# wgurecky/CORRLA_RS

Measured on AMD Instinct MI355X. Metric: RSVD GFLOP/s on 16k x 16k f32 rank-128, higher is better.
Workload: dtype f32

## Files before the change

### corrla_rs_amd/csrc/hip_backend.hpp

```cpp
#pragma once
#include <hip/hip_runtime.h>
#include <rccl/rccl.h>

#include <cmath>
#include <cstdio>
#include <cstdlib>
#include <cstring>
#include <limits>
#include <random>
#include <string>
#include <type_traits>
#include <vector>

#include "core_svd_plan.hpp"
#include "driver.hpp"
#include "hip_kernels.hpp"
#include "tsqr_kernels.hpp"
#include "jacobi_mc_kernels.hpp"
#include "ata_kernels.hpp"
#include "tall_kernels.hpp"
#include "mixed_kernels.hpp"
#include "grad_kernels.hpp"
#include "knn2_kernels.hpp"
#include "grad_wide_kernels.hpp"
#include "spmm_kernels.hpp"

namespace corrla {

#define CORRLA_HIP(call)                                                                                       \
  do {                                                                                                         \
    hipError_t e_ = (call);                                                                                    \
    if (e_ != hipSuccess)                                                                                      \
      throw Error(ST_EHIP, std::string(#call) + " failed: " + hipGetErrorString(e_) + " (" __FILE__ ":" +       \
                               std::to_string(__LINE__) + ")");                                                \
  } while (0)
#define CORRLA_NCCL(call)                                                                                      \
  do {                                                                                                         \
    ncclResult_t r_ = (call);                                                                                  \
    if (r_ != ncclSuccess) throw Error(ST_ECOMM, std::string(#call) + " failed: " + ncclGetErrorString(r_));   \
  } while (0)

inline int env_int(const char* name, int dflt) {
  const char* v = std::getenv(name);
  return v && *v ? std::atoi(v) : dflt;
}

template <class T>
struct NcclType;
template <>
struct NcclType<float> {
  static constexpr ncclDataType_t v = ncclFloat;
};
template <>
struct NcclType<double> {
  static constexpr ncclDataType_t v = ncclDouble;
};

class HipDev {
 public:
  int device = 0;
  int num_cus = 256;
  hipStream_t stream = nullptr;
  ncclComm_t comm = nullptr;
  int comm_rank = 0, comm_size = 1;
  int n_collectives = 0;
  double collective_bytes = 0;

  explicit HipDev(int dev_ordinal) : device(dev_ordinal) {
    int count = 0;
    if (hipGetDeviceCount(&count) != hipSuccess || count <= 0)
      throw Error(ST_ENODEV, "no HIP device visible (libcorrla_rsvd has no CPU fallback)");
    if (dev_ordinal < 0 || dev_ordinal >= count) throw Error(ST_EINVAL, "device ordinal out of range");
    CORRLA_HIP(hipSetDevice(device));
    hipDeviceProp_t prop;
    CORRLA_HIP(hipGetDeviceProperties(&prop, device));
    if (std::strncmp(prop.gcnArchName, "gfx950", 6) != 0)
      throw Error(ST_ENODEV, std::string("device is ") + prop.gcnArchName + ", this library is built for gfx950 only");
    num_cus = prop.multiProcessorCount;
    CORRLA_HIP(hipStreamCreateWithFlags(&stream, hipStreamNonBlocking));
    CORRLA_HIP(hipMalloc(&zero_page_, 256));
    CORRLA_HIP(hipHostMalloc(&pinned_, kPinnedBytes, hipHostMallocDefault));
    for (auto& e : events_) CORRLA_HIP(hipEventCreate(&e));
    CORRLA_HIP(hipMemsetAsync(zero_page_, 0, 256, stream));
    set_lds_limits();
    {
      std::random_device rd;
      entropy_ = ((uint64_t)rd() << 32) ^ (uint64_t)rd();
    }
    no_device_chol_ = env_int("CORRLA_HOST_CHOL", 0) != 0;
    jmc_min_l_ = env_int("CORRLA_JMC_MIN_L", 96);
    jmc_max_b_ = std::min(32, std::max(2, env_int("CORRLA_JMC_MAX_B", 24)));
    robust_passes_ = std::max(2, env_int("CORRLA_ROBUST_PASSES", 2));
    robust_qr_ = env_int("CORRLA_DEVICE_ROBUST_QR", 1) != 0;
    gemm_debug_flags_ = env_int("CORRLA_GEMM_DEBUG", 0);
    gemm_knobs_.split_nn = env_int("CORRLA_SPLIT_NN", 0);
    gemm_knobs_.split_tn = env_int("CORRLA_SPLIT_TN", 0);
    gemm_knobs_.mw = env_int("CORRLA_MW", 0);
    gemm_knobs_.xcd_remap = env_int("CORRLA_GEMM_XCD", 1);
    gemm_knobs_.tall_min_rows = env_int("CORRLA_TALL_MIN_ROWS", 65536);
    gemm_knobs_.persist_max_tiles = env_int("CORRLA_GEMM_PERSIST_TILES", 16);
    gemm_knobs_.f64_waves = env_int("CORRLA_F64_WAVES", 8);
    if (const char* e = std::getenv("CORRLA_MIXED_MIN_WORK")) gemm_knobs_.mixed_min_work = std::atof(e);
    gemm_knobs_.even_blocks = env_int("CORRLA_EVEN_BLOCKS", 0) != 0;
    gemm_knobs_.no_gram_alias = env_int("CORRLA_NO_GRAM_ALIAS", 0) != 0;
    gemm_knobs_.no_rotate = env_int("CORRLA_GEMM_NO_ROTATE", 0) != 0;
    gemm_knobs_.mixed_split = env_int("CORRLA_MIXED_SPLIT", 0);
  }
  ~HipDev() {
    (void)hipSetDevice(device);
    if (stream) (void)hipStreamSynchronize(stream);
    if (comm) (void)ncclCommDestroy(comm);
    for (auto& c : chunks_) (void)hipFree(c.p);
    for (auto& c : zchunks_) (void)hipFree(c.p);
    if (zero_page_) (void)hipFree(zero_page_);
    if (pinned_) (void)hipHostFree(pinned_);
    for (auto& e : events_)
      if (e) (void)hipEventDestroy(e);
    for (auto& e : ev_pool_) (void)hipEventDestroy(e);
    if (stream) (void)hipStreamDestroy(stream);
  }
  HipDev(const HipDev&) = delete;
  HipDev& operator=(const HipDev&) = delete;

  int nranks() const { return comm_size; }

  uint64_t fresh_seed(bool rank_invariant) {
    uint64_t z = (rank_invariant ? 0x5eedull : entropy_) + 0x9e3779b97f4a7c15ull * (uint64_t)(++(rank_invariant ? calls_sharded_ : calls_));
    z = (z ^ (z >> 30)) * 0xbf58476d1ce4e5b9ull;
    z = (z ^ (z >> 27)) * 0x94d049bb133111ebull;
    z ^= z >> 31;
    return z ? z : 0x5eedull;
  }

  void comm_init(const void* id128, int rank, int nranks_) {
    CORRLA_HIP(hipSetDevice(device));
    ncclUniqueId id;
    static_assert(sizeof(ncclUniqueId) <= CORRLA_UNIQUE_ID_BYTES, "unique id size");
    std::memcpy(&id, id128, sizeof(id));
    if (comm) {
      (void)ncclCommDestroy(comm);
      comm = nullptr;
    }
    CORRLA_NCCL(ncclCommInitRank(&comm, nranks_, id, rank));
    comm_rank = rank;
    comm_size = nranks_;
  }
  void comm_info(int* rank_out, int* nranks_out) {
    if (!comm) {
      *rank_out = 0;
      *nranks_out = 0;
      return;
    }
    CORRLA_NCCL(ncclCommUserRank(comm, rank_out));
    CORRLA_NCCL(ncclCommCount(comm, nranks_out));
  }

  void begin_call() {
    CORRLA_HIP(hipSetDevice(device));
    events_set_[0] = events_set_[1] = events_set_[2] = false;
    n_collectives = 0;
    collective_bytes = 0;
    marks_.clear();
    ev_used_ = 0;
    phase_mark(nullptr);
    for (auto& c : chunks_) c.used = 0;
    sp_scratch_ = nullptr;
    sp_scratch_bytes_ = 0;
    for (auto& c : zchunks_) {
      c.zeroed = std::min<size_t>(c.used, (size_t)256 << 20);
      c.used = 0;
      if (c.zeroed) CORRLA_HIP(hipMemsetAsync(c.p, 0, c.zeroed, stream));
    }
// ... 337 lines not shown
    sync();
    for (size_t i = 0; i < n; ++i) host[i] = (double)tmp[i];
  }
  template <class T>
  void upload_skinny(const double* host, int64_t rows, int64_t cols, int64_t ld_host, Skinny<T>& dst) {
    const size_t n = (size_t)dst.ld * dst.cols_alloc;
    std::vector<T> heap;
    T* tmp = (T*)pinned_;
    if (n * sizeof(T) > kPinnedBytes) {
      heap.resize(n);
      tmp = heap.data();
    }
    sync();
    std::memset(tmp, 0, n * sizeof(T));
    for (int64_t j = 0; j < cols; ++j)
      for (int64_t i = 0; i < rows; ++i) tmp[(size_t)j * dst.ld + i] = (T)host[(size_t)j * ld_host + i];
    CORRLA_HIP(hipMemcpyAsync(dst.p, tmp, n * sizeof(T), hipMemcpyHostToDevice, stream));
    if (!heap.empty()) sync();
  }
  template <class T>
  void upload_skinny_native(const T* host, int64_t ld_host, Skinny<T>& dst) {
    h2d_2d(dst.p, dst.ld, host, ld_host, dst.rows, dst.cols);
  }
  template <class T>
  void copy_in_skinny(const T* src_dev, int64_t ld_src, Skinny<T>& dst) {
    CORRLA_HIP(hipMemcpy2DAsync(dst.p, (size_t)dst.ld * sizeof(T), src_dev, (size_t)ld_src * sizeof(T),
                                (size_t)dst.rows * sizeof(T), (size_t)dst.cols, hipMemcpyDeviceToDevice, stream));
  }
  template <class T>
  void copy_skinny(const Skinny<T>& src, Skinny<T>& dst) {
    CORRLA_HIP(hipMemcpyAsync(dst.p, src.p, (size_t)src.ld * src.cols_alloc * sizeof(T), hipMemcpyDeviceToDevice, stream));
  }
  template <class T>
  void copy_cols(const Skinny<T>& src, Skinny<T>& dst, int64_t c0, int64_t n) {
    if (src.ld != dst.ld) throw Error(ST_EINVAL, "internal: copy_cols needs equal leading dimensions");
    if (n > 0)
      CORRLA_HIP(hipMemcpyAsync(dst.p + c0 * dst.ld, src.p, (size_t)n * src.ld * sizeof(T), hipMemcpyDeviceToDevice, stream));
  }
  template <class T>
  void sub_inplace(Skinny<T>& y, const Skinny<T>& p) {
    const int64_t n = y.ld * std::min(y.cols_alloc, p.cols_alloc);
    const int blocks = (int)std::min<int64_t>(4096, std::max<int64_t>(1, (n + 255) / 256));
    hipLaunchKernelGGL((k::sub_kernel<T>), dim3(blocks), dim3(256), 0, stream, y.p, (const T*)p.p, n);
    CORRLA_HIP(hipGetLastError());
  }
  template <class T>
  void zero_cols(Skinny<T>& s, int64_t c0, int64_t c1) {
    if (c1 > c0) memset_zero(s.p + c0 * s.ld, (size_t)(c1 - c0) * s.ld * sizeof(T));
  }
  template <class T>
  void store_values(const T* host_src, int64_t n, T* dst, bool dst_is_host) {
    if (dst_is_host) {
      std::memcpy(dst, host_src, sizeof(T) * n);
    } else {
      CORRLA_HIP(hipMemcpyAsync(dst, host_src, sizeof(T) * n, hipMemcpyHostToDevice, stream));
      sync();
    }
  }
  template <class T>
  void copy_values_out(const T* src_dev, int64_t n, T* dst, bool dst_is_host) {
    CORRLA_HIP(hipMemcpyAsync(dst, src_dev, sizeof(T) * n, dst_is_host ? hipMemcpyDeviceToHost : hipMemcpyDeviceToDevice,
                              stream));
    if (dst_is_host) sync();
  }
  template <class T>
  bool device_chol_fits(int64_t l) const {
    return l <= 4096 && k::chol_inv_fits((int)l, sizeof(T)) && !no_device_chol_;
  }
  template <class T>
  bool device_chol_blocked_fits(int64_t l) const {
    const int64_t n1 = round_up((l + 1) / 2, (int64_t)4);
    return l > 8 && l <= 4096 && k::chol_inv_fits((int)n1, sizeof(T)) && !no_device_chol_;
  }
  template <class T>
  void copy_block(const Skinny<T>& src, int64_t r0, int64_t c0, int64_t rows, int64_t cols, Skinny<T>& dst, int64_t dr0,
                  int64_t dc0) {
    if (rows <= 0 || cols <= 0) return;
    CORRLA_HIP(hipMemcpy2DAsync(dst.p + dc0 * dst.ld + dr0, (size_t)dst.ld * sizeof(T), src.p + c0 * src.ld + r0,
                                (size_t)src.ld * sizeof(T), (size_t)rows * sizeof(T), (size_t)cols, hipMemcpyDeviceToDevice,
                                stream));
  }
  template <class T>
  void chol_inv(const Skinny<T>& g, int64_t r, T piv_rel, Skinny<T>& m_out, void* st_dev, int slot) {
    hipLaunchKernelGGL((k::chol_inv_kernel<T>), dim3(1), dim3(k::chol_inv_threads((int)r)),
                       k::chol_inv_lds_bytes((int)r, sizeof(T)), stream, (const T*)g.p, g.ld, (int)r, piv_rel, m_out.p,
                       m_out.ld, (k::CholStatus*)st_dev + slot);
    CORRLA_HIP(hipGetLastError());
  }
  void set_run_if(const int* p) { run_if_ = p; }
  int robust_passes() const { return robust_passes_; }
  void set_robust_passes(int n) { robust_passes_ = n; }
  bool svd_more_sweeps() {
    if (jmc_extra_sweeps_ >= 24) return false;
    jmc_extra_sweeps_ += 8;
    jmc_sweeps_hint_ = 0;
    return true;
  }
  bool svd_force_v() {
    if (jmc_force_v_) return false;
    jmc_force_v_ = true;
    return true;
  }
  void svd_sweeps_used(int n) { jmc_sweeps_hint_ = std::max(jmc_sweeps_hint_ - 1, n); }
  int* alloc_flags(int n) { return (int*)alloc_zeroed(sizeof(int) * (size_t)std::max(n, 1)); }
  void* alloc_zeroed_bytes(size_t bytes) { return alloc_zeroed(bytes); }
  void read_bytes(const void* dev_p, size_t bytes, void* host) {
    CORRLA_HIP(hipMemcpyAsync(host, dev_p, bytes, hipMemcpyDeviceToHost, stream));
    sync();
  }
  template <class T>
  void poison_entry(Skinny<T>& s, int64_t i, int64_t j, int kind) {
    hipLaunchKernelGGL((k::poison_entry_kernel<T>), dim3(1), dim3(1), 0, stream, s.p + j * s.ld + i, kind);
    CORRLA_HIP(hipGetLastError());
  }
  struct ArenaMark {
    std::vector<size_t> used, zused;
  };
  ArenaMark arena_mark() const {
    ArenaMark mk;
    for (const auto& c : chunks_) mk.used.push_back(c.used);
    for (const auto& c : zchunks_) mk.zused.push_back(c.used);
    return mk;
  }
  void arena_rewind(const ArenaMark& mk) {
    sp_scratch_ = nullptr;
    sp_scratch_bytes_ = 0;
    for (size_t i = 0; i < chunks_.size(); ++i) chunks_[i].used = i < mk.used.size() ? mk.used[i] : 0;
    for (size_t i = 0; i < zchunks_.size(); ++i) {
      Chunk& c = zchunks_[i];
      const size_t keep = i < mk.zused.size() ? mk.zused[i] : 0;
      if (c.used > keep) CORRLA_HIP(hipMemsetAsync((char*)c.p + keep, 0, c.used - keep, stream));
      c.zeroed = std::max(c.zeroed, c.used);
      c.used = keep;
    }
  }
  int sharded_handshake(int local_status) {
    if (comm_size <= 1 && !(comm && env_int("CORRLA_FORCE_ALLREDUCE", 0))) return local_status;
    if (!comm) throw Error(ST_ECOMM, "communicator not initialised");
    double h[8] = {(double)local_status, (double)robust_passes_, (double)jmc_extra_sweeps_, (double)jmc_sweeps_hint_,
                   jmc_force_v_ ? 1.0 : 0.0, 0.0, 0.0, 0.0};
    double* d = (double*)alloc_bytes(sizeof(h));
    CORRLA_HIP(hipMemcpyAsync(d, h, sizeof(h), hipMemcpyHostToDevice, stream));
    CORRLA_NCCL(ncclAllReduce(d, d, 8, ncclDouble, ncclMax, comm, stream));
    ++n_collectives;
    collective_bytes += sizeof(h);
    CORRLA_HIP(hipMemcpyAsync(h, d, sizeof(h), hipMemcpyDeviceToHost, stream));
    sync();
    robust_passes_ = (int)h[1];
    jmc_extra_sweeps_ = (int)h[2];
    jmc_sweeps_hint_ = (int)h[3];
    jmc_force_v_ = h[4] != 0.0;
    return (int)h[0];
  }
  void read_flags(const int* dev_p, int n, int* host) {
    CORRLA_HIP(hipMemcpyAsync(host, dev_p, sizeof(int) * (size_t)n, hipMemcpyDeviceToHost, stream));
    sync();
  }
  template <class T>
  bool device_qr_robust_fits(int64_t l) const {
    return robust_qr_ && (device_chol_fits<T>(l) || device_chol_blocked_fits<T>(l));
  }
  bool qr_inplace_fits(int64_t l) const { return col_blocking(l).nblk == 1; }
  template <class T>
  void* alloc_inspect() { return alloc_zeroed(sizeof(k::GramInspect<T>)); }
  template <class T>
  const void* inspect_shift_ptr(const void* insp) const { return &((const k::GramInspect<T>*)insp)->shift; }
  template <class T>
  void gram_inspect(Skinny<T>& g, int64_t l, float shift_rel, int shift_mode, void* insp) {
    hipLaunchKernelGGL((k::gram_inspect_kernel<T>), dim3(1), dim3(1024), 0, stream, g.p, g.ld, (int)l, shift_rel, shift_mode,
                       (k::GramInspect<T>*)insp, run_if_);
    CORRLA_HIP(hipGetLastError());
  }
  template <class T>
  void combine_need(int* need, const void* insp, const int* na, const int* nb) {
    hipLaunchKernelGGL((k::combine_need_kernel<T>), dim3(1), dim3(1), 0, stream, need, (const k::GramInspect<T>*)insp, na, nb,
                       run_if_);
    CORRLA_HIP(hipGetLastError());
  }
  template <class T>
  void chol_inv_robust(const Skinny<T>& g, int64_t r, T piv_rel, float shift_rel, int shift_mode, float null_excess,
                       Skinny<T>& m_out, void* st_dev, int slot, int* need_next, int* null_mask,
                       const void* abs_shift = nullptr, float need_ratio = 0.f) {
    k::CholRobust rb{shift_rel, shift_mode, null_excess, need_next, null_mask, run_if_, need_ratio, abs_shift};
    hipLaunchKernelGGL((k::chol_inv_kernel<T>), dim3(1), dim3(k::chol_inv_threads((int)r)),
                       k::chol_inv_lds_bytes((int)r, sizeof(T)), stream, (const T*)g.p, g.ld, (int)r, piv_rel, m_out.p,
                       m_out.ld, (k::CholStatus*)st_dev + slot, rb);
    CORRLA_HIP(hipGetLastError());
  }
  template <class T>
  void apply_inplace(Skinny<T>& y, int64_t l, const Skinny<T>& m) {
    Skinny<T> out = y.view_cols(l);
    Skinny<T> mv = m.view_cols(l);
    mv.rows = l;
    launch_gemm<T>(true, as_rowmajor_transposed(y, l), mv, out, (const T*)nullptr);
  }
  template <class T>
  void refill_null(Skinny<T>& y, int64_t l, const int* null_mask, uint64_t seed) {
    const int bx = (int)std::min<int64_t>(64, (y.rows + 255) / 256);
    hipLaunchKernelGGL((k::refill_null_kernel<T>), dim3((unsigned)std::max(bx, 1), (unsigned)l), dim3(256), 0, stream, y.p, y.ld,
                       y.rows, (int)l, null_mask, seed, run_if_);
    CORRLA_HIP(hipGetLastError());
  }

  void read_chol_status(const void* st_dev, int n, int* fail, float* min_ratio, float* dev_i) {
    static_assert(sizeof(k::CholStatus) == 32, "driver.hpp assumes 32-byte status records");
    static_assert(k::kNeedNonFinite == kFlagNonFinite && k::kNeedNullCols == kFlagNullCols, "need_next bits: kernels vs driver");
    std::vector<k::CholStatus> h((size_t)std::max(n, 1));
    CORRLA_HIP(hipMemcpyAsync(h.data(), st_dev, sizeof(k::CholStatus) * n, hipMemcpyDeviceToHost, stream));
    sync();
    for (int i = 0; i < n; ++i) {
      fail[i] = h[i].fail;
      min_ratio[i] = h[i].min_ratio;
      dev_i[i] = h[i].dev_i;
      if (env_int("CORRLA_DEBUG", 0) >= 2)
        std::fprintf(stderr, "[corrla] chol_inv[%d]: fail %d min_ratio %.3g dev_i %.3g clk %lld wall %lld (%.0f MHz)\n", i,
                     h[i].fail, h[i].min_ratio, h[i].dev_i, h[i].clk, h[i].wall,
                     h[i].wall > 0 ? 100.0 * (double)h[i].clk / (double)h[i].wall : 0.0);
    }
  }

  template <class T>
  void inv_sqrt_series(Skinny<T>& g, int64_t r, Skinny<T>& m_out) {
    Skinny<T> e2 = alloc_skinny<T>(r, r), e3 = alloc_skinny<T>(r, r);
    if (e2.ld != g.ld || m_out.ld != g.ld) throw Error(ST_EINVAL, "internal: series operands must share a leading dimension");
    dim3 grid((unsigned)((r + 63) / 64), (unsigned)r);
    hipLaunchKernelGGL((k::series_prep_kernel<T>), grid, dim3(64), 0, stream, g.p, g.ld, (int)r);
    Big<T> eb;
    eb.p = g.p;
    eb.rows = r;
    eb.cols = r;
    eb.ld = g.ld;
    eb.cols_readable = g.ld;
    Skinny<T> gv = g.view_cols(r);
    gv.rows = r;
    gemm_nn(eb, gv, e2, (const T*)nullptr);
    gemm_nn(eb, e2, e3, (const T*)nullptr);
    memset_zero(m_out.p, (size_t)m_out.ld * m_out.cols_alloc * sizeof(T));
    hipLaunchKernelGGL((k::series_combine_kernel<T>), grid, dim3(64), 0, stream, (const T*)g.p, (const T*)e2.p,
                       (const T*)e3.p, g.ld, (int)r, m_out.p, m_out.ld);
    CORRLA_HIP(hipGetLastError());
  }

  bool hh_wy_ = env_int("CORRLA_HH_WY", 1) != 0;
  template <class T>
  size_t hh_panel_lds(int rows, int l) const {
    return hh_wy_ ? k::hh_wy_lds_bytes(rows, l, sizeof(T)) : k::hh_lds_bytes(rows, l, sizeof(T));
  }
  template <class T>
  bool householder_fits(int64_t l) const {
    return l >= 1 && l <= 4096 && hh_panel_lds<T>((int)(2 * l), (int)l) <= (size_t)160 * 1024 && 2 * l <= 64 * k::kHhMaxRowsPerLane;
  }
  template <class T>
  struct HhState {
    int64_t m = 0;
    int l = 0, nleaf = 0, levels = 0, max_rows = 0;
    std::vector<int> n_at;
    std::vector<T*> rbuf, cbuf, taub, vbuf, tbuf;
    T* r_root() const { return rbuf[levels]; }
  };
  template <class T>
  HhState<T> householder_up(Skinny<T>& y, Skinny<T>& tmp) {
    HhState<T> h;
    const int64_t m = y.rows;
    const int l = (int)y.cols;
    if (m < l) throw Error(ST_EINVAL, "householder_thin_q: fewer rows than columns");
    if (!householder_fits<T>(l)) throw Error(ST_EINVAL, "householder_thin_q: panel does not fit in LDS");
    const int64_t br = 2 * (int64_t)l;
    const int64_t nleaf64 = m <= br ? 1 : (m + br - 1) / br;
    if (nleaf64 > 0x3fffffff) throw Error(ST_EINVAL, "householder_thin_q: too many panels");
// ... 398 lines not shown
    hipEvent_t e = ev_pool_[ev_used_++];
    CORRLA_HIP(hipEventRecord(e, stream));
    marks_.push_back({e, slot});
  }
  void phase_forget() {
    for (auto& m_ : marks_) m_.slot = nullptr;
  }
  void phase_resolve(double* total) {
    for (size_t i = 1; i < marks_.size(); ++i) {
      float ms = 0.f;
      if (hipEventElapsedTime(&ms, marks_[i - 1].ev, marks_[i].ev) != hipSuccess) {
        (void)hipGetLastError();
        continue;
      }
      if (marks_[i].slot) *marks_[i].slot += (double)ms;
    }
    if (total && marks_.size() >= 2) {
      float ms = 0.f;
      if (hipEventElapsedTime(&ms, marks_.front().ev, marks_.back().ev) == hipSuccess)
        *total = (double)ms;
      else
        (void)hipGetLastError();
    }
    marks_.clear();
  }

  void event_mark(int i) {
    CORRLA_HIP(hipEventRecord(events_[i], stream));
    events_set_[i] = true;
  }
  double event_elapsed_ms(int i, int j) {
    if (!events_set_[i] || !events_set_[j]) return 0.0;
    float ms = 0.f;
    if (hipEventElapsedTime(&ms, events_[i], events_[j]) != hipSuccess) {
      (void)hipGetLastError();
      return 0.0;
    }
    return (double)ms;
  }

  template <class F>
  double time_on_stream(int reps, F&& f) {
    hipEvent_t e0, e1;
    CORRLA_HIP(hipEventCreate(&e0));
    CORRLA_HIP(hipEventCreate(&e1));
    f();
    CORRLA_HIP(hipEventRecord(e0, stream));
    for (int i = 0; i < reps; ++i) f();
    CORRLA_HIP(hipEventRecord(e1, stream));
    CORRLA_HIP(hipEventSynchronize(e1));
    float ms = 0.f;
    CORRLA_HIP(hipEventElapsedTime(&ms, e0, e1));
    (void)hipEventDestroy(e0);
    (void)hipEventDestroy(e1);
    return (double)ms / reps;
  }

 private:
  struct Chunk {
    void* p = nullptr;
    size_t size = 0, used = 0;
    size_t zeroed = 0;
  };
  std::vector<Chunk> chunks_;
  std::vector<Chunk> zchunks_;
  void* sp_scratch_ = nullptr;
  size_t sp_scratch_bytes_ = 0;
  void* zero_page_ = nullptr;
  void* pinned_ = nullptr;
  hipEvent_t events_[3] = {nullptr, nullptr, nullptr};
  bool events_set_[3] = {false, false, false};
  struct PhaseMark {
    hipEvent_t ev;
    double* slot;
  };
  std::vector<hipEvent_t> ev_pool_;
  size_t ev_used_ = 0;
  std::vector<PhaseMark> marks_;
  static constexpr size_t kPinnedBytes = (size_t)8 << 20;
  int gemm_debug_flags_ = 0;
  GemmKnobs gemm_knobs_;
  uint64_t entropy_ = 0, calls_ = 0, calls_sharded_ = 0;
  bool no_device_chol_ = false;
  int jmc_min_l_ = 96, jmc_max_b_ = 24, jmc_local_ = 1;
  const int* run_if_ = nullptr;
  bool phase_events_ = true;
  bool robust_qr_ = true;
  int robust_passes_ = 2;
  int jmc_extra_sweeps_ = 0, jmc_sweeps_hint_ = 0;
  bool jmc_force_v_ = false;

  static void check_grid(const dim3& g) {
    if (g.y > 65535u || g.z > 65535u) throw Error(ST_EINVAL, "problem too large for the launch grid");
  }

  static void lds_limit(const void* fn, size_t bytes) {
    CORRLA_HIP(hipFuncSetAttribute(fn, hipFuncAttributeMaxDynamicSharedMemorySize, (int)bytes));
  }
  static void set_lds_limits() {
    constexpr size_t kMax = k::kLdsMaxBytes;
    set_lds_limits_typed<float>();
    set_lds_limits_typed<double>();
    set_ata_limits<2>();
    set_ata_limits<4>();
    set_ata_limits<8>();
    set_mixed_limits<2, false>();
    set_mixed_limits<2, true>();
    set_mixed_limits<3, false>();
    set_mixed_limits<3, true>();
    lds_limit((const void*)k::knn_kernel, kMax);
    lds_limit((const void*)k::knn_mfma_kernel<4, 4>, kMax);
    lds_limit((const void*)k::knn_mfma_kernel<4, 8>, kMax);
    lds_limit((const void*)k::knn_mfma_kernel<4, 16>, kMax);
    lds_limit((const void*)k::knn_mfma_kernel<2, 4>, kMax);
    lds_limit((const void*)k::knn_mfma_kernel<2, 8>, kMax);
    lds_limit((const void*)k::knn_mfma_kernel<2, 16>, kMax);
    lds_limit((const void*)k::knn2_kernel<1>, k::k2_lds_bytes(1));
    lds_limit((const void*)k::knn2_kernel<2>, k::k2_lds_bytes(2));
    lds_limit((const void*)k::grad_fit_kernel, kMax);
    lds_limit((const void*)k::grad_fit_lin_kernel<1>, kMax);
    lds_limit((const void*)k::grad_fit_lin_kernel<2>, kMax);
    lds_limit((const void*)k::grad_fit_lin_kernel<3>, kMax);
    lds_limit((const void*)k::grad_fit_lin_kernel<4>, kMax);
    lds_limit((const void*)k::grad_fit_lin_kernel<5>, kMax);
    lds_limit((const void*)k::knn_wide_kernel, k::ws_lds_bytes());
    lds_limit((const void*)k::grad_fit_wide_kernel, k::wf_lds_bytes());
  }
  template <class T>
  static void set_lds_limits_typed() {
    constexpr size_t kMax = k::kLdsMaxBytes;
    for_each_nt<kMaxColTiles>([](auto nt) { set_gemm_limits<T, decltype(nt)::value>(); });
    for_each_nt<sizeof(T) == 4 ? 6 : 4>([](auto nct) {
      lds_limit((const void*)k::tall_gram_kernel<T, decltype(nct)::value>, k::gram_lds_bytes(nct, (int)sizeof(T)));
    });
    lds_limit((const void*)k::hh_leaf_factor_kernel<T, false>, kMax);
    lds_limit((const void*)k::hh_tree_factor_kernel<T, false>, kMax);
    lds_limit((const void*)k::hh_tree_apply_kernel<T, false>, kMax);
    lds_limit((const void*)k::hh_leaf_apply_kernel<T, false>, kMax);
    lds_limit((const void*)k::hh_leaf_factor_kernel<T, true>, kMax);
    lds_limit((const void*)k::hh_tree_factor_kernel<T, true>, kMax);
    lds_limit((const void*)k::hh_tree_apply_kernel<T, true>, kMax);
    lds_limit((const void*)k::hh_leaf_apply_kernel<T, true>, kMax);
    constexpr int kBigE = sizeof(T) == 4 ? 20 : 18;
    lds_limit((const void*)k::jacobi_ring_w_kernel<T, 8, 8>, kMax);
    lds_limit((const void*)k::jacobi_ring_w_kernel<T, 12, 8>, kMax);
    lds_limit((const void*)k::jacobi_ring_w_kernel<T, 16, 8>, kMax);
    lds_limit((const void*)k::jacobi_ring_w_kernel<T, kBigE, 8>, kMax);
    lds_limit((const void*)k::jacobi_block_round_kernel<T>, kMax);
    for_each_nt<9>([](auto nc) { lds_limit((const void*)k::jmc_step_kernel<T, decltype(nc)::value, 16>, k::kLdsMaxBytes); });
  }
  template <class T, int NT>
  static void set_gemm_limits() {
    lds_limit((const void*)k::gemm_nn_kernel<T, 1, NT>, k::gemm_lds_bytes(1, NT));
    lds_limit((const void*)k::gemm_tn_kernel<T, 1, NT>, k::gemm_lds_bytes(1, NT));
    lds_limit((const void*)k::gemm_nn_kernel<T, 2, NT>, k::gemm_lds_bytes(2, NT));
    lds_limit((const void*)k::gemm_tn_kernel<T, 2, NT>, k::gemm_lds_bytes(2, NT));
    if constexpr (NT <= 8) lds_limit((const void*)k::gemm_nn_kernel<T, 2, NT, true>, 3 * k::big_tile_bytes(2));
    if constexpr (std::is_same<T, double>::value) {
      lds_limit((const void*)k::gemm_nn_kernel<T, 1, NT, false, 8>, k::gemm_lds_bytes(2, NT));
      lds_limit((const void*)k::gemm_tn_kernel<T, 1, NT, 8>, k::gemm_lds_bytes(2, NT));
    }
  }
  template <int NK>
  static void set_ata_limits() {
    for_each_nt<5>([](auto nct) { lds_limit((const void*)k::ata_fused_kernel<NK, decltype(nct)::value>, k::ata_lds_bytes(NK, nct)); });
  }
  template <int NP, bool TN>
  static void set_mixed_limits() {
    for_each_nt<kMaxColTiles>([](auto nt) {
      lds_limit((const void*)k::gemm_bf16s_kernel<decltype(nt)::value, NP, TN>, k::mx_lds_bytes(nt, NP));
    });
  }
  template <class T>
  GemmShape gemm_shape(bool tn, const Big<T>& r, const Skinny<T>& x, const Skinny<T>& out, int np) const {
    auto aligned = [](const void* p) { return (uintptr_t)p % 16 == 0; };
    GemmShape s;
    s.tn = tn;
    s.esz = (int)sizeof(T);
    s.r = {r.rows, r.cols, r.ld, r.cols_readable, 0, false, aligned(r.p)};
    s.x = {x.rows, x.cols, x.ld, 0, x.cols_alloc, x.external, aligned(x.p)};
    s.out = {out.rows, out.cols, out.ld, 0, out.cols_alloc, out.external, aligned(out.p)};
    s.same = (const void*)r.p == (const void*)x.p;
    s.np = np;
    s.num_cus = num_cus;
    return s;
  }
  template <class T>
  GemmPlan plan_gemm(bool tn, const Big<T>& r, const Skinny<T>& x, const Skinny<T>& out, int np) const {
    const GemmPlan p = gemm_plan(gemm_shape(tn, r, x, out, np), gemm_knobs_);
    if (p.error) throw Error(ST_EINVAL, p.error);
    return p;
  }
  template <int MAX, int N = 1, class F>
  static void with_nt(int n, const F& f) {
    if constexpr (N < MAX) {
      if (n > N) return with_nt<MAX, N + 1>(n, f);
    }
    if (n != N) throw Error(ST_EINVAL, "internal: no kernel instantiation for " + std::to_string(n));
    f(std::integral_constant<int, N>{});
  }
  template <int MAX, int N = 1, class F>
  static void for_each_nt(const F& f) {
    f(std::integral_constant<int, N>{});
    if constexpr (N < MAX) for_each_nt<MAX, N + 1>(f);
  }
  template <class T>
  void slab_reduce(const SlabReducePlan& rp, const T* slab, int64_t stride, T* out, int64_t ld, const T* scale, const int* run_if) {
    if (rp.kind == SlabReduce::none) return;
    const dim3 grid(rp.grid[0], rp.grid[1]);
    if (rp.kind == SlabReduce::deep)
      hipLaunchKernelGGL((k::slab_reduce_deep_kernel<T>), grid, dim3(256), 0, stream, slab, stride, rp.slabs, out, ld, rp.rows,
                         rp.cols, scale, run_if);
    else
      hipLaunchKernelGGL((k::slab_reduce_kernel<T>), grid, dim3(256), 0, stream, slab, stride, rp.slabs, out, ld, rp.rows, rp.cols,
                         scale, run_if);
    CORRLA_HIP(hipGetLastError());
  }
// ... 71 lines not shown
```

### corrla_rs_amd/csrc/hip_kernels.hpp

```cpp
#pragma once
#include <hip/hip_runtime.h>

#include <limits>
#include <stdint.h>

#include <type_traits>

#include "gemm_plan.hpp"

namespace corrla {
namespace k {

typedef float f32x4 __attribute__((ext_vector_type(4)));
typedef double f64x4 __attribute__((ext_vector_type(4)));
typedef double f64x2 __attribute__((ext_vector_type(2)));

#ifndef CORRLA_F32_BIG_IS_A
#define CORRLA_F32_BIG_IS_A true
#endif
template <class T>
struct MT;
template <>
struct MT<float> {
  typedef f32x4 acc_t;
// ... 1422 lines not shown
struct CholStatus {
  int fail;
  float min_ratio;
  float dev_i;
  float gmax;
  long long clk, wall;
};
constexpr int kNeedNonFinite = 2;
constexpr int kNeedNullCols = 4;
struct CholRobust {
  float shift_rel;
  int shift_mode;
  float null_excess;
  int* need_next;
  int* null_mask;
  const int* run_if;
  float need_ratio;
  const void* abs_shift;
};
template <class T>
struct GramInspect {
  T shift;
  int shifted;
  int bad;
  float d2;
  float gmax;
};
template <class T>
__global__ __launch_bounds__(1024) void gram_inspect_kernel(T* g, int64_t ld, int l, float shift_rel, int shift_mode,
                                                            GramInspect<T>* out, const int* run_if) {
  if (run_if && *run_if == 0) return;
  __shared__ float rd[16], rg[16];
  __shared__ int sbad;
  const int tid = threadIdx.x;
  if (tid == 0) sbad = 0;
  float dv = 0.f, gm = 0.f;
  int bad = 0;
  for (int idx = tid; idx < l * l; idx += 1024) {
    const int j = idx / l, i = idx - j * l;
    const T x = g[(int64_t)j * ld + i];
    if (!((float)fabs(x) < 3.0e38f)) bad = 1;
    dv = fmaxf(dv, (float)fabs(x - (i == j ? (T)1 : (T)0)));
    if (i == j) gm = fmaxf(gm, (float)x);
  }
  for (int off = 32; off > 0; off >>= 1) {
    dv = fmaxf(dv, __shfl_down(dv, off, 64));
    gm = fmaxf(gm, __shfl_down(gm, off, 64));
  }
  __syncthreads();
  if ((tid & 63) == 0) {
    rd[tid >> 6] = dv;
    rg[tid >> 6] = gm;
  }
  if (bad) sbad = 1;
  __syncthreads();
  dv = 0.f;
  gm = 0.f;
  for (int i = 0; i < 16; ++i) {
    dv = fmaxf(dv, rd[i]);
    gm = fmaxf(gm, rg[i]);
  }
  const bool shifted = !sbad && gm > 0.f && shift_rel > 0.f && (shift_mode == 1 || (shift_mode == 0 && dv > 0.25f));
  const T sh = shifted ? (T)shift_rel * (T)gm : (T)0;
  if (shifted)
    for (int i = tid; i < l; i += 1024) g[(int64_t)i * ld + i] += sh;
  if (tid == 0) {
    out->shift = sh;
    out->shifted = shifted ? 1 : 0;
    out->bad = sbad;
    out->d2 = dv;
    out->gmax = gm;
  }
}
template <class T>
__global__ void combine_need_kernel(int* need, const GramInspect<T>* insp, const int* na, const int* nb, const int* run_if) {
  if (run_if && *run_if == 0) return;
  const int sub = *na | *nb;
  const int bad = (insp && insp->bad) ? kNeedNonFinite : 0;
  const int need1 = ((insp && (insp->shifted || insp->bad || insp->d2 > 0.05f)) || sub) ? 1 : 0;
  *need = need1 | bad | (sub & (kNeedNonFinite | kNeedNullCols));
}
template <class T>
__host__ __device__ constexpr int chol_inv_max_threads() { return sizeof(T) == 8 ? 768 : 1024; }
template <class T>
__global__ __launch_bounds__(chol_inv_max_threads<T>()) void chol_inv_kernel(const T* __restrict__ g, int64_t ldg, int r, T piv_rel, T* m,
                                                        int64_t ldm, CholStatus* st, CholRobust rq = CholRobust{0.f, 0, 0.f, nullptr, nullptr, nullptr, 0.f, nullptr}) {
  if (rq.run_if && *rq.run_if == 0) return;
  const bool robust = rq.need_next != nullptr;
  extern __shared__ __attribute__((aligned(16))) char smem[];
  const int nt = (r + 3) >> 2, r4 = nt * 4;
  T* rowbuf = (T*)smem;
  T* colbuf = rowbuf + 2 * r4;
  T* diag0 = colbuf + 2 * r4;
  T* dis = diag0 + r4;
  float* red = (float*)(dis + r4);
  const int tid = threadIdx.x, nwave = blockDim.x >> 6;
  const int ntri = nt * (nt + 1) / 2;
  const bool own = tid < ntri;
  int ti = 0, tk = 0;
  if (own) {
    const int e = ntri - 1 - tid;
    int c = (int)((sqrtf(8.f * (float)e + 1.f) - 1.f) * 0.5f);
    while (c * (c + 1) / 2 > e) --c;
    while ((c + 1) * (c + 2) / 2 <= e) ++c;
    ti = nt - 1 - c;
    tk = nt - 1 - (e - c * (c + 1) / 2);
  }
  const int i0 = 4 * ti, k0 = 4 * tk;
  T v[4][4], w[4][4];
  float dv = 0.f, gm = 0.f;
  int bad = 0;
#pragma unroll
  for (int aa = 0; aa < 4; ++aa)
#pragma unroll
    for (int b = 0; b < 4; ++b) {
      const int i = min(i0 + aa, r - 1), k = min(k0 + b, r - 1);
      v[aa][b] = g[(int64_t)k * ldg + i];
    }
#pragma unroll
  for (int aa = 0; aa < 4; ++aa)
#pragma unroll
    for (int b = 0; b < 4; ++b) {
      const int i = i0 + aa, k = k0 + b;
      const bool in = own && i < r && k < r;
      const T x = in ? v[aa][b] : (T)0;
      if (in) {
        if (!((float)fabs(x) < 3.0e38f)) bad = 1;
        dv = fmaxf(dv, (float)fabs(x - (i == k ? (T)1 : (T)0)));
        if (i == k) gm = fmaxf(gm, (float)x);
      }
      v[aa][b] = x;
      w[aa][b] = (own && i == k && i < r) ? (T)1 : (T)0;
    }
  for (int idx = tid; idx < 4 * r4; idx += blockDim.x) rowbuf[idx] = (T)0;
  if (own && ti == tk) {
#pragma unroll
    for (int aa = 0; aa < 4; ++aa) diag0[i0 + aa] = v[aa][aa];
  }
  for (int off = 32; off > 0; off >>= 1) {
    dv = fmaxf(dv, __shfl_down(dv, off, 64));
    gm = fmaxf(gm, __shfl_down(gm, off, 64));
  }
  if ((tid & 63) == 0) {
    red[tid >> 6] = dv;
    red[16 + (tid >> 6)] = gm;
  }
  bad = __syncthreads_or(bad);
  float d2 = 0.f, g2 = 0.f;
  for (int i = 0; i < nwave; ++i) {
    d2 = fmaxf(d2, red[i]);
    g2 = fmaxf(g2, red[16 + i]);
  }
  int fl = bad ? 3 : (!(g2 > 0.f) ? 2 : 0);
  float min_ratio = 1.f;
  int nnull = 0;
  if (robust && fl == 2) {
    for (int j = tid; j < r; j += blockDim.x) rq.null_mask[j] = 1;
    if (own) {
#pragma unroll
      for (int aa = 0; aa < 4; ++aa)
#pragma unroll
        for (int b = 0; b < 4; ++b) {
          const int i = i0 + aa, k = k0 + b;
          if (i <= k && k < r) m[(int64_t)k * ldm + i] = (T)0;
        }
    }
    if (tid == 0) {
      *rq.need_next = 1 | kNeedNullCols;
      st->fail = 0;
      st->min_ratio = 0.f;
      st->dev_i = d2;
      st->gmax = 0.f;
      st->clk = 0;
      st->wall = 0;
    }
    return;
  }
  const long long clk0 = clock64(), wall0 = wall_clock64();
  const float series_tol = sizeof(T) == 4 ? 2.0e-4f : 1.0e-8f;
  if (fl == 0 && d2 <= series_tol) {
    if (own) {
#pragma unroll
      for (int aa = 0; aa < 4; ++aa)
#pragma unroll
        for (int b = 0; b < 4; ++b) {
          const int i = i0 + aa, k = k0 + b;
          if (i < r && k < r) {
            const T val = (i == k ? (T)1 : (T)0) - (T)0.5 * (v[aa][b] - (i == k ? (T)1 : (T)0));
            m[(int64_t)k * ldm + i] = val;
            m[(int64_t)i * ldm + k] = val;
          }
        }
    }
    if (robust)
      for (int j = tid; j < r; j += blockDim.x) rq.null_mask[j] = 0;
    if (tid == 0) {
      if (robust) *rq.need_next = 0;
      st->fail = 0;
      st->min_ratio = 1.f;
      st->dev_i = d2;
      st->gmax = g2;
      st->clk = 0;
      st->wall = 0;
    }
    return;
  }
  const T pre_sh = rq.abs_shift ? *(const T*)rq.abs_shift : (T)0;
  const bool shifted = rq.abs_shift ? pre_sh > (T)0
                                    : (robust && rq.shift_rel > 0.f && (rq.shift_mode == 1 || (rq.shift_mode == 0 && d2 > 0.25f)));
  const T sh = rq.abs_shift ? pre_sh : (shifted ? (T)rq.shift_rel * (T)g2 : (T)0);
  if (fl == 0 && shifted && !rq.abs_shift) {
    if (own && ti == tk) {
#pragma unroll
      for (int aa = 0; aa < 4; ++aa)
        if (i0 + aa < r) v[aa][aa] += sh;
    }
  }
  if (fl == 0) {
    typedef T V4 __attribute__((ext_vector_type(4)));
    for (int tj = 0; tj < nt && fl == 0; ++tj) {
#pragma unroll
      for (int aj = 0; aj < 4; ++aj) {
        const int j = 4 * tj + aj;
        if (j >= r) break;
        T* rb = rowbuf + (j & 1) * r4;
        T* cb = colbuf + (j & 1) * r4;
        if (own && ti == tj) *(V4*)&rb[k0] = V4{v[aj][0], v[aj][1], v[aj][2], v[aj][3]};
        if (own && tk == tj) *(V4*)&cb[i0] = V4{w[0][aj], w[1][aj], w[2][aj], w[3][aj]};
        __syncthreads();
        const T d = rb[j];
        const T g0 = diag0[j];
        const V4 rk4 = *(const V4*)&rb[k0];
        const V4 ri4 = *(const V4*)&rb[i0];
        const V4 ci4 = *(const V4*)&cb[i0];
        if (!(d > piv_rel * g0) || !(g0 > (T)0) ||
            (shifted && rq.null_excess > 0.f && !(d - sh > (T)rq.null_excess * sh))) {
          if (!robust) {
            fl = 1;
            break;
          }
          ++nnull;
          if (tid == 0) dis[j] = (T)0;
          continue;
        }
        if (tid < 64) {
          min_ratio = fminf(min_ratio, (float)d * fast_rcp((float)g0));
          if (tid == 0) {
            T rs = fast_rsqrt(d);
            rs = rs * ((T)1.5 - (T)0.5 * d * rs * rs);
            dis[j] = rs;
          }
        }
        if (own && tk >= tj) {
          T rinv = fast_rcp(d);
          rinv = rinv * ((T)2 - d * rinv);
          T rk[4];
#pragma unroll
          for (int q = 0; q < 4; ++q) rk[q] = rk4[q] * rinv;
          if (ti >= tj) {
            T ri[4] = {ri4[0], ri4[1], ri4[2], ri4[3]};
            if (ti == tj) {
#pragma unroll
              for (int q = 0; q < 4; ++q) ri[q] = (q > aj) ? ri[q] : (T)0;
            }
#pragma unroll
            for (int aa = 0; aa < 4; ++aa)
#pragma unroll
              for (int b = 0; b < 4; ++b) v[aa][b] -= ri[aa] * rk[b];
          }
          if (ti <= tj) {
            T ci[4] = {ci4[0], ci4[1], ci4[2], ci4[3]};
            if (ti == tj) {
#pragma unroll
              for (int q = 0; q < 4; ++q) ci[q] = (q <= aj) ? ci[q] : (T)0;
            }
            if (tk == tj) {
#pragma unroll
              for (int q = 0; q < 4; ++q) rk[q] = (q > aj) ? rk[q] : (T)0;
            }
#pragma unroll
            for (int aa = 0; aa < 4; ++aa)
#pragma unroll
              for (int b = 0; b < 4; ++b) w[aa][b] -= ci[aa] * rk[b];
          }
        }
      }
    }
  }
  const long long clk1 = clock64(), wall1 = wall_clock64();
  __syncthreads();
  if (robust && fl == 0)
    for (int j = tid; j < r; j += blockDim.x) rq.null_mask[j] = dis[j] == (T)0 ? 1 : 0;
  if (own) {
#pragma unroll
    for (int aa = 0; aa < 4; ++aa)
#pragma unroll
      for (int b = 0; b < 4; ++b) {
        const int i = i0 + aa, k = k0 + b;
        if (i <= k && k < r)
          m[(int64_t)k * ldm + i] = (fl == 0) ? w[aa][b] * dis[k] : ((i == k && fl == 1) ? (T)1 : (T)0);
      }
  }
  if (tid == 0) {
    if (robust) {
      int need;
      if (rq.need_ratio > 0.f)
        need = (nnull > 0 || min_ratio < rq.need_ratio || fl != 0) ? 1 : 0;
      else
        need = (nnull > 0 || d2 > 0.05f || (shifted && !rq.abs_shift) || fl != 0) ? 1 : 0;
      *rq.need_next = need | (fl == 3 ? kNeedNonFinite : 0) | (nnull > 0 ? kNeedNullCols : 0);
    }
    st->fail = fl;
    st->min_ratio = nnull > 0 ? 0.f : min_ratio;
    st->dev_i = d2;
    st->gmax = g2;
    st->clk = clk1 - clk0;
    st->wall = wall1 - wall0;
  }
}
template <class T>
__global__ void refill_null_kernel(T* y, int64_t ld, int64_t m, int l, const int* null_mask, uint64_t seed, const int* run_if) {
  if (run_if && *run_if == 0) return;
  const int j = blockIdx.y;
  if (j >= l || null_mask[j] == 0) return;
  const T sc = (T)rsqrt((double)m);
  for (int64_t i = (int64_t)blockIdx.x * blockDim.x + threadIdx.x; i < m; i += (int64_t)gridDim.x * blockDim.x)
    y[(int64_t)j * ld + i] = sc * normal_from_index<T>((uint64_t)(i * l + j), seed);
}
__host__ __device__ inline int chol_inv_threads(int r) {
  const int nt = (r + 3) / 4;
  return ((nt * (nt + 1) / 2 + 63) / 64) * 64;
}
__host__ __device__ inline size_t chol_inv_lds_bytes(int r, size_t esz) {
  return (size_t)6 * (((size_t)r + 3) / 4 * 4) * esz + 32 * sizeof(float) + 64;
}
__host__ __device__ inline bool chol_inv_fits(int r, size_t esz) {
  return r >= 1 && chol_inv_threads(r) <= (esz == 8 ? 768 : 1024);
}

template <class T>
__global__ void series_prep_kernel(T* g, int64_t ld, int r) {
  const int i = blockIdx.x * blockDim.x + threadIdx.x, j = blockIdx.y;
  if (i < r && j < r && i == j) g[(int64_t)j * ld + i] -= (T)1;
}
template <class T>
__global__ void series_combine_kernel(const T* e1, const T* e2, const T* e3, int64_t ld, int r, T* m, int64_t ldm) {
  const int i = blockIdx.x * blockDim.x + threadIdx.x, j = blockIdx.y;
  if (i >= r || j >= r) return;
  const int64_t o = (int64_t)j * ld + i;
  m[(int64_t)j * ldm + i] = (i == j ? (T)1 : (T)0) - (T)0.5 * e1[o] + (T)0.375 * e2[o] - (T)0.3125 * e3[o];
}

template <class T>
__global__ __launch_bounds__(1024) void core_finite_check_kernel(const T* __restrict__ c, int64_t ld, int l, CholStatus* st, int* bad_out) {
  int bad = 0;
  for (int idx = threadIdx.x; idx < l * l; idx += 1024) {
    const int j = idx / l, i = idx - j * l;
    if (!((float)fabs(c[(int64_t)j * ld + i]) < 3.0e38f)) bad = 1;
  }
  bad = __syncthreads_or(bad);
  if (threadIdx.x == 0 && bad) {
    if (st) st->fail = 3;
    if (bad_out) *bad_out = 1;
  }
}
template <class T>
__global__ void poison_entry_kernel(T* p, int kind) {
  *p = kind == 2 ? std::numeric_limits<T>::infinity() : std::numeric_limits<T>::quiet_NaN();
}

template <class T>
__global__ void fill_const_kernel(T* p, int64_t n, T v) {
  for (int64_t i = (int64_t)blockIdx.x * blockDim.x + threadIdx.x; i < n; i += (int64_t)gridDim.x * blockDim.x) p[i] = v;
}
template <class T>
__global__ void center_kernel(const T* in, int64_t rows, int64_t cols, int64_t ldi, const T* mu, int along_cols, T* out,
                              int64_t ldo) {
  const int64_t c = (int64_t)blockIdx.x * blockDim.x + threadIdx.x;
  if (c >= cols) return;
  const T mc = along_cols ? mu[c] : (T)0;
  for (int64_t r = blockIdx.y; r < rows; r += gridDim.y) {
    const T m_ = along_cols ? mc : mu[r];
    out[r * ldo + c] = in[r * ldi + c] - m_;
  }
}

template <class T>
__global__ __launch_bounds__(256) void wcolsum_partial_kernel(const T* __restrict__ x, int64_t ld, int64_t rows,
                                                              const T* __restrict__ w, double* partial, int ncols) {
  __shared__ double red[256];
  const int c = blockIdx.y;
  const int64_t per = (rows + gridDim.x - 1) / gridDim.x;
  const int64_t r0 = (int64_t)blockIdx.x * per, r1 = min(rows, r0 + per);
  double s = 0.0;
  for (int64_t r = r0 + threadIdx.x; r < r1; r += 256) s += (w ? (double)w[r] : 1.0) * (double)x[(int64_t)c * ld + r];
  red[threadIdx.x] = s;
  __syncthreads();
  for (int off = 128; off > 0; off >>= 1) {
    if ((int)threadIdx.x < off) red[threadIdx.x] += red[threadIdx.x + off];
    __syncthreads();
  }
  if (threadIdx.x == 0) partial[(int64_t)blockIdx.x * ncols + c] = red[0];
}
template <class T>
__global__ void wcolsum_final_kernel(const double* partial, int nblk, int ncols, T* v) {
  const int c = blockIdx.x * blockDim.x + threadIdx.x;
  if (c >= ncols) return;
  double s = 0.0;
  for (int b = 0; b < nblk; ++b) s += partial[(int64_t)b * ncols + c];
  v[c] = (T)s;
}
template <class T>
__global__ void rank1_sub_kernel(T* out, int64_t ld, int64_t rows, const T* __restrict__ u, const T* __restrict__ v,
                                 const T* __restrict__ scale) {
  const int64_t i = (int64_t)blockIdx.x * blockDim.x + threadIdx.x;
  if (i >= rows) return;
  const T sc = scale ? *scale : (T)1;
// ... 95 lines not shown
```

Baseline: 94830.

## Add MFMA-based blocked Cholesky-inverse fast path for f32 Gram matrices

Adds a blocked 16x16-tile Cholesky factorization and triangular inverse for f32, computed in LDS with MFMA 16x16x4 instructions inside the single-block chol_inv kernel. It is enabled by default for the first slot(s) of chol_inv and chol_inv_robust. If any pivot falls below a threshold it falls back to the original scalar path after reloading the register tiles. The aim is to cut the serial latency of the single-workgroup Cholesky step in the CholeskyQR pipeline. In exchange it needs much more LDS, adds pivot-based fallback logic, and may change numerics slightly.

```diff
diff --git a/corrla_rs_amd/csrc/hip_backend.hpp b/corrla_rs_amd/csrc/hip_backend.hpp
--- a/corrla_rs_amd/csrc/hip_backend.hpp
+++ b/corrla_rs_amd/csrc/hip_backend.hpp
@@ -88,6 +88,7 @@
       entropy_ = ((uint64_t)rd() << 32) ^ (uint64_t)rd();
     }
     no_device_chol_ = env_int("CORRLA_HOST_CHOL", 0) != 0;
+    chol_fast_ = env_int("CORRLA_CHOL_FAST", 1) != 0;
     jmc_min_l_ = env_int("CORRLA_JMC_MIN_L", 96);
     jmc_max_b_ = std::min(32, std::max(2, env_int("CORRLA_JMC_MAX_B", 24)));
     robust_passes_ = std::max(2, env_int("CORRLA_ROBUST_PASSES", 2));
@@ -591,9 +592,11 @@
   }
   template <class T>
   void chol_inv(const Skinny<T>& g, int64_t r, T piv_rel, Skinny<T>& m_out, void* st_dev, int slot) {
+    const bool fast = chol_fast_ && slot == 0;
     hipLaunchKernelGGL((k::chol_inv_kernel<T>), dim3(1), dim3(k::chol_inv_threads((int)r)),
-                       k::chol_inv_lds_bytes((int)r, sizeof(T)), stream, (const T*)g.p, g.ld, (int)r, piv_rel, m_out.p,
-                       m_out.ld, (k::CholStatus*)st_dev + slot);
+                       k::chol_inv_lds_bytes((int)r, sizeof(T), fast), stream, (const T*)g.p, g.ld, (int)r, piv_rel, m_out.p,
+                       m_out.ld, (k::CholStatus*)st_dev + slot, k::CholRobust{0.f, 0, 0.f, nullptr, nullptr, nullptr, 0.f, nullptr},
+                       fast ? 1 : 0);
     CORRLA_HIP(hipGetLastError());
   }
   void set_run_if(const int* p) { run_if_ = p; }
@@ -691,9 +694,10 @@
                        Skinny<T>& m_out, void* st_dev, int slot, int* need_next, int* null_mask,
                        const void* abs_shift = nullptr, float need_ratio = 0.f) {
     k::CholRobust rb{shift_rel, shift_mode, null_excess, need_next, null_mask, run_if_, need_ratio, abs_shift};
+    const bool fast = chol_fast_ && slot < (abs_shift ? 2 : 1);
     hipLaunchKernelGGL((k::chol_inv_kernel<T>), dim3(1), dim3(k::chol_inv_threads((int)r)),
-                       k::chol_inv_lds_bytes((int)r, sizeof(T)), stream, (const T*)g.p, g.ld, (int)r, piv_rel, m_out.p,
-                       m_out.ld, (k::CholStatus*)st_dev + slot, rb);
+                       k::chol_inv_lds_bytes((int)r, sizeof(T), fast), stream, (const T*)g.p, g.ld, (int)r, piv_rel, m_out.p,
+                       m_out.ld, (k::CholStatus*)st_dev + slot, rb, fast ? 1 : 0);
     CORRLA_HIP(hipGetLastError());
   }
   template <class T>
@@ -1258,6 +1262,7 @@
   GemmKnobs gemm_knobs_;
   uint64_t entropy_ = 0, calls_ = 0, calls_sharded_ = 0;
   bool no_device_chol_ = false;
+  bool chol_fast_ = true;
   int jmc_min_l_ = 96, jmc_max_b_ = 24, jmc_local_ = 1;
   const int* run_if_ = nullptr;
   bool phase_events_ = true;
@@ -1309,6 +1314,7 @@
     for_each_nt<sizeof(T) == 4 ? 6 : 4>([](auto nct) {
       lds_limit((const void*)k::tall_gram_kernel<T, decltype(nct)::value>, k::gram_lds_bytes(nct, (int)sizeof(T)));
     });
+    lds_limit((const void*)k::chol_inv_kernel<T>, k::chol_inv_lds_bytes(sizeof(T) == 4 ? 176 : 152, sizeof(T), true));
     lds_limit((const void*)k::hh_leaf_factor_kernel<T, false>, kMax);
     lds_limit((const void*)k::hh_tree_factor_kernel<T, false>, kMax);
     lds_limit((const void*)k::hh_tree_apply_kernel<T, false>, kMax);
diff --git a/corrla_rs_amd/csrc/hip_kernels.hpp b/corrla_rs_amd/csrc/hip_kernels.hpp
--- a/corrla_rs_amd/csrc/hip_kernels.hpp
+++ b/corrla_rs_amd/csrc/hip_kernels.hpp
@@ -1528,9 +1528,158 @@
 }
 template <class T>
 __host__ __device__ constexpr int chol_inv_max_threads() { return sizeof(T) == 8 ? 768 : 1024; }
+constexpr int kCfLd = 17;
+constexpr int kCfTile = 16 * kCfLd;
+constexpr int kCholFastMinR = 16;
+constexpr float kCholFastMinPivot = 1.0f / 1024.0f;
+__host__ __device__ inline size_t chol_fast_lds_bytes(int r) {
+  const size_t nb = ((size_t)r + 15) / 16;
+  return (nb * (nb + 1) / 2 + nb) * kCfTile * sizeof(float);
+}
+__device__ inline float cf_readlane(float x, int lane) {
+  return __int_as_float(__builtin_amdgcn_readlane(__float_as_int(x), lane));
+}
+typedef float cf_f4 __attribute__((ext_vector_type(4)));
+__device__ inline cf_f4 cf_tile_mma(cf_f4 acc, const float* pa, int sa, int ka, float as, const float* pb, int lane) {
+  const int x = lane & 15, kq = lane >> 4;
+  float a[4], b[4];
+#pragma unroll
+  for (int s = 0; s < 4; ++s) {
+    a[s] = pa[x * sa + (4 * s + kq) * ka];
+    b[s] = pb[(4 * s + kq) * kCfLd + x];
+  }
+#pragma unroll
+  for (int s = 0; s < 4; ++s) acc = __builtin_amdgcn_mfma_f32_16x16x4f32(as * a[s], b[s], acc, 0, 0, 0);
+  return acc;
+}
+__device__ inline cf_f4 cf_tile_load(const float* t, int lane) {
+  const int col = lane & 15, row = 4 * (lane >> 4);
+  return cf_f4{t[row * kCfLd + col], t[(row + 1) * kCfLd + col], t[(row + 2) * kCfLd + col], t[(row + 3) * kCfLd + col]};
+}
+__device__ inline void cf_tile_store(float* t, int lane, cf_f4 v) {
+  const int col = lane & 15, row = 4 * (lane >> 4);
+#pragma unroll
+  for (int q = 0; q < 4; ++q) t[(row + q) * kCfLd + col] = v[q];
+}
+__device__ inline bool chol_fast_f32(const float* __restrict__ g, int64_t ldg, int r, float piv_rel, float sh_add, float g2,
+                                     const float* diag0, int* flag, float* tiles, float* m, int64_t ldm, float& min_ratio) {
+  const int tid = threadIdx.x, lane = tid & 63, wave = tid >> 6, nwave = blockDim.x >> 6;
+  const int nb = (r + 15) >> 4, ntile = nb * (nb + 1) / 2;
+  float* rowp = tiles + (size_t)ntile * kCfTile;
+  const int ea = lane & 15, eb = lane >> 4;
+  for (int t = wave, c = 0; t < ntile; t += nwave) {
+    while ((c + 1) * (c + 2) / 2 <= t) ++c;
+    const int i = t - c * (c + 1) / 2;
+    float* tp = tiles + (size_t)t * kCfTile;
+    float x[4];
+#pragma unroll
+    for (int q = 0; q < 4; ++q) {
+      const int row = 16 * i + ea, col = 16 * c + eb + 4 * q;
+      const int rr = min(min(row, col), r - 1), cc = min(max(row, col), r - 1);
+      x[q] = g[(int64_t)cc * ldg + rr];
+    }
+#pragma unroll
+    for (int q = 0; q < 4; ++q) {
+      const int row = 16 * i + ea, col = 16 * c + eb + 4 * q;
+      const bool in = row < r && col < r;
+      float val = in ? x[q] : (row == col ? 1.f : 0.f);
+      if (in && row == col) val += sh_add;
+      tp[ea * kCfLd + eb + 4 * q] = val;
+    }
+  }
+  if (tid == 0) *flag = 0;
+  __syncthreads();
+  float mr = 1.f;
+  for (int p = 0; p < nb; ++p) {
+    float* tpp = tiles + (size_t)(p * (p + 1) / 2 + p) * kCfTile;
+    if (wave == 0) {
+      float cc[16], vv[16];
+#pragma unroll
+      for (int i = 0; i < 16; ++i) {
+        cc[i] = tpp[i * kCfLd + ea];
+        vv[i] = (i == ea) ? 1.f : 0.f;
+      }
+      const float g0l = diag0[min(16 * p + ea, r - 1)];
+      bool ok = true;
+#pragma unroll
+      for (int k = 0; k < 16; ++k) {
+        const float d = cf_readlane(cc[k], k);
+        if (16 * p + k < r) {
+          const float g0 = cf_readlane(g0l, k);
+          if (!(d > piv_rel * g0) || !(g0 > 0.f) || !(d > kCholFastMinPivot * g2)) ok = false;
+          mr = fminf(mr, d * fast_rcp(g0));
+        }
+        float rs = fast_rsqrt(d);
+        rs = rs * (1.5f - 0.5f * d * rs * rs);
+        const float rk = cc[k] * rs;
+        const float rkm = ea > k ? rk : 0.f;
+#pragma unroll
+        for (int i = k + 1; i < 16; ++i) cc[i] -= cf_readlane(rk, i) * rk;
+#pragma unroll
+        for (int i = 0; i <= k; ++i) {
+          const float xi = vv[i] * rs;
+          const float s = cf_readlane(xi, k);
+          vv[i] = (ea == k) ? xi : vv[i] - s * rkm;
+        }
+      }
+      if (ok) {
+        if (lane < 16) {
+#pragma unroll
+          for (int i = 0; i < 16; ++i) tpp[i * kCfLd + ea] = vv[i];
+        }
+      } else if (lane == 0) {
+        *flag = 1;
+      }
+    }
+    __syncthreads();
+    if (*flag) return false;
+    const int nrow = nb - 1 - p;
+    for (int t = wave; t < nrow + p; t += nwave) {
+      if (t < nrow) {
+        const int c = p + 1 + t;
+        const float* gpc = tiles + (size_t)(c * (c + 1) / 2 + p) * kCfTile;
+        cf_tile_store(rowp + (size_t)c * kCfTile, lane, cf_tile_mma(cf_f4{0.f, 0.f, 0.f, 0.f}, tpp, 1, kCfLd, 1.f, gpc, lane));
+      } else {
+        const int i = t - nrow;
+        float* vip = tiles + (size_t)(p * (p + 1) / 2 + i) * kCfTile;
+        cf_tile_store(vip, lane, cf_tile_mma(cf_f4{0.f, 0.f, 0.f, 0.f}, vip, kCfLd, 1, 1.f, tpp, lane));
+      }
+    }
+    __syncthreads();
+    if (nrow == 0) break;
+    int t = 0;
+    for (int c = p + 1; c < nb; ++c) {
+      const float* rpc = rowp + (size_t)c * kCfTile;
+      for (int i = 0; i <= c; ++i, ++t) {
+        if (t % nwave != wave) continue;
+        float* tic = tiles + (size_t)(c * (c + 1) / 2 + i) * kCfTile;
+        if (i <= p) {
+          const cf_f4 acc = i < p ? cf_tile_load(tic, lane) : cf_f4{0.f, 0.f, 0.f, 0.f};
+          cf_tile_store(tic, lane, cf_tile_mma(acc, tiles + (size_t)(p * (p + 1) / 2 + i) * kCfTile, kCfLd, 1, -1.f, rpc, lane));
+        } else {
+          cf_tile_store(tic, lane, cf_tile_mma(cf_tile_load(tic, lane), rowp + (size_t)i * kCfTile, 1, kCfLd, -1.f, rpc, lane));
+        }
+      }
+    }
+    __syncthreads();
+  }
+  for (int t = wave, c = 0; t < ntile; t += nwave) {
+    while ((c + 1) * (c + 2) / 2 <= t) ++c;
+    const int i = t - c * (c + 1) / 2;
+    const float* tp = tiles + (size_t)t * kCfTile;
+#pragma unroll
+    for (int q = 0; q < 4; ++q) {
+      const int row = 16 * i + ea, col = 16 * c + eb + 4 * q;
+      if (row <= col && col < r) m[(int64_t)col * ldm + row] = tp[ea * kCfLd + eb + 4 * q];
+    }
+  }
+  min_ratio = mr;
+  return true;
+}
 template <class T>
 __global__ __launch_bounds__(chol_inv_max_threads<T>()) void chol_inv_kernel(const T* __restrict__ g, int64_t ldg, int r, T piv_rel, T* m,
-                                                        int64_t ldm, CholStatus* st, CholRobust rq = CholRobust{0.f, 0, 0.f, nullptr, nullptr, nullptr, 0.f, nullptr}) {
+                                                        int64_t ldm, CholStatus* st, CholRobust rq = CholRobust{0.f, 0, 0.f, nullptr, nullptr, nullptr, 0.f, nullptr},
+                                                        int fast = 0) {
   if (rq.run_if && *rq.run_if == 0) return;
   const bool robust = rq.need_next != nullptr;
   extern __shared__ __attribute__((aligned(16))) char smem[];
@@ -1655,6 +1804,50 @@
   const bool shifted = rq.abs_shift ? pre_sh > (T)0
                                     : (robust && rq.shift_rel > 0.f && (rq.shift_mode == 1 || (rq.shift_mode == 0 && d2 > 0.25f)));
   const T sh = rq.abs_shift ? pre_sh : (shifted ? (T)rq.shift_rel * (T)g2 : (T)0);
+  if constexpr (sizeof(T) == 4) {
+    if (fast && fl == 0 && rq.null_excess == 0.f && r >= kCholFastMinR) {
+      int* fflag = (int*)(red + 32);
+      float mr = 1.f;
+      if (chol_fast_f32(g, ldg, r, piv_rel, (shifted && !rq.abs_shift) ? sh : 0.f, g2, diag0, fflag, (float*)(fflag + 16), m, ldm,
+                        mr)) {
+        const long long clk1 = clock64(), wall1 = wall_clock64();
+        if (robust)
+          for (int j = tid; j < r; j += blockDim.x) rq.null_mask[j] = 0;
+        if (tid == 0) {
+          if (robust) {
+            int need;
+            if (rq.need_ratio > 0.f)
+              need = mr < rq.need_ratio ? 1 : 0;
+            else
+              need = (d2 > 0.05f || (shifted && !rq.abs_shift)) ? 1 : 0;
+            *rq.need_next = need;
+          }
+          st->fail = 0;
+          st->min_ratio = mr;
+          st->dev_i = d2;
+          st->gmax = g2;
+          st->clk = clk1 - clk0;
+          st->wall = wall1 - wall0;
+        }
+        return;
+      }
+#pragma unroll
+      for (int aa = 0; aa < 4; ++aa)
+#pragma unroll
+        for (int b = 0; b < 4; ++b) {
+          const int i = min(i0 + aa, r - 1), k = min(k0 + b, r - 1);
+          v[aa][b] = g[(int64_t)k * ldg + i];
+        }
+#pragma unroll
+      for (int aa = 0; aa < 4; ++aa)
+#pragma unroll
+        for (int b = 0; b < 4; ++b) {
+          const int i = i0 + aa, k = k0 + b;
+          v[aa][b] = (own && i < r && k < r) ? v[aa][b] : (T)0;
+          w[aa][b] = (own && i == k && i < r) ? (T)1 : (T)0;
+        }
+    }
+  }
   if (fl == 0 && shifted && !rq.abs_shift) {
     if (own && ti == tk) {
 #pragma unroll
@@ -1777,8 +1970,10 @@
   const int nt = (r + 3) / 4;
   return ((nt * (nt + 1) / 2 + 63) / 64) * 64;
 }
-__host__ __device__ inline size_t chol_inv_lds_bytes(int r, size_t esz) {
-  return (size_t)6 * (((size_t)r + 3) / 4 * 4) * esz + 32 * sizeof(float) + 64;
+__host__ __device__ inline bool chol_inv_fast_fits(int r, size_t esz) { return esz == 4 && r >= kCholFastMinR; }
+__host__ __device__ inline size_t chol_inv_lds_bytes(int r, size_t esz, bool fast = false) {
+  return (size_t)6 * (((size_t)r + 3) / 4 * 4) * esz + 32 * sizeof(float) + 64 +
+         (fast && chol_inv_fast_fits(r, esz) ? chol_fast_lds_bytes(r) : 0);
 }
 __host__ __device__ inline bool chol_inv_fits(int r, size_t esz) {
   return r >= 1 && chol_inv_threads(r) <= (esz == 8 ? 768 : 1024);
```

Measured after the change: 94540. Within noise of the previous version (-0.3%).
